# rpp0/gr-lora

Hardware: NVIDIA H100
Metric: LoRa symbols/s (dechirp+FFT+argmax) (higher is better)
Workload: dtype f32

## Files before the change

### gr_lora_b200/csrc/host_emul.cu

```cuda
#include "cuda_owned.h"
#include "k1_fft.cuh"
#include "k1_llr.cuh"
#include "k1_warp.cuh"
#include "k1_group.cuh"
#include "k1_sf10.cuh"
#include "k1_rows.cuh"
#include "int_chain.cuh"
#include "rx_stream.cuh"
#include "rx_sync.cuh"
#include "tx_channel.cuh"
#include "tx_encode.cuh"

#include <algorithm>
#include <cstring>
#include <vector>

template <int D>
static int k1_emulate_d(int sf, const lb::K1Args &a, uint32_t *bins, float *mags) {
    switch (sf) {
    case 7: lb::k1_emulate<7, D>(a, bins, mags); break;
    case 8: lb::k1_emulate<8, D>(a, bins, mags); break;
    case 9: lb::k1_emulate<9, D>(a, bins, mags); break;
    case 10: lb::k1_emulate<10, D>(a, bins, mags); break;
    case 11: lb::k1_emulate<11, D>(a, bins, mags); break;
    case 12: lb::k1_emulate<12, D>(a, bins, mags); break;
    default: return -1;
    }
    return 0;
}

template <int D>
static int k1_llr_emulate_d(int sf, const lb::K1Args &a, bool reduced, float *llrs, uint32_t *bins) {
    switch (sf) {
    case 7: lb::k1_llr_emulate<7, D>(a, reduced, llrs, bins); break;
    case 8: lb::k1_llr_emulate<8, D>(a, reduced, llrs, bins); break;
    case 9: lb::k1_llr_emulate<9, D>(a, reduced, llrs, bins); break;
    case 10: lb::k1_llr_emulate<10, D>(a, reduced, llrs, bins); break;
    case 11: lb::k1_llr_emulate<11, D>(a, reduced, llrs, bins); break;
    case 12: lb::k1_llr_emulate<12, D>(a, reduced, llrs, bins); break;
    default: return -1;
    }
    return 0;
}

extern "C" {

int lb_k1_emulate_osr(int sf, int osr, const float2 *x, size_t n_symbols, const float2 *chirp, const float2 *tw, uint32_t *bins,
                      float *mags) {
    const lb::K1Args a{x, chirp, tw, n_symbols};
    return osr == 8 ? k1_emulate_d<8>(sf, a, bins, mags) : osr == 2 ? k1_emulate_d<2>(sf, a, bins, mags) : -1;
}

int lb_k1_emulate(int sf, const float2 *x, size_t n_symbols, const float2 *chirp, const float2 *tw,
                  uint32_t *bins, float *mags) {
    return lb_k1_emulate_osr(sf, 8, x, n_symbols, chirp, tw, bins, mags);
}

int lb_k1_llr_emulate_osr(int sf, int osr, const float2 *x, size_t n_symbols, const float2 *chirp, const float2 *tw, int reduced,
                          float *llrs, uint32_t *bins) {
    const lb::K1Args a{x, chirp, tw, n_symbols};
    return osr == 8 ? k1_llr_emulate_d<8>(sf, a, reduced != 0, llrs, bins) : osr == 2 ? k1_llr_emulate_d<2>(sf, a, reduced != 0, llrs, bins) : -1;
}

int lb_k1_llr_emulate(int sf, const float2 *x, size_t n_symbols, const float2 *chirp, const float2 *tw, int reduced, float *llrs,
                      uint32_t *bins) {
    return lb_k1_llr_emulate_osr(sf, 8, x, n_symbols, chirp, tw, reduced, llrs, bins);
}

int lb_k1_emulate_warp_sf7(const float2 *x, size_t n_symbols, const float2 *chirp, const float2 *tw, uint32_t *bins, float *mags) {
    lb::K1Args a{x, chirp, tw, n_symbols};
    lb::w7_emulate(a, bins, mags);
    return 0;
}

int lb_k1_emulate_group(int sf, const float2 *x, size_t n_symbols, const float2 *chirp, const float2 *tw, uint32_t *bins, float *mags) {
    lb::K1Args a{x, chirp, tw, n_symbols};
    switch (sf) {
    case 8: lb::g_emulate<8>(a, bins, mags); break;
    case 9: lb::g_emulate<9>(a, bins, mags); break;
    case 10: lb::s10_emulate(a, bins, mags); break;
    default: return -1;
    }
    return 0;
}

int lb_k1_emulate_rows(int sf, const float2 *x, size_t n_symbols, const float2 *chirp, const float2 *tw, uint32_t *bins, float *mags) {
    lb::K1Args a{x, chirp, tw, n_symbols};
    if (sf == 11) lb::r_emulate<11>(a, bins, mags);
    else if (sf == 12) lb::r_emulate<12>(a, bins, mags);
    else return -1;
    return 0;
}


void lb_emul_philox4x32_10(const uint32_t *ctr, const uint32_t *key, uint32_t *out) {
    uint32_t c[4] = {ctr[0], ctr[1], ctr[2], ctr[3]};
    lb::philox4x32_10(c, key[0], key[1]);
    for (int i = 0; i < 4; i++) out[i] = c[i];
}

void lb_emul_atan2f(const float *y, const float *x, float *out, size_t n) {
    for (size_t i = 0; i < n; i++) out[i] = lb::lb_atan2f(y[i], x[i]);
}

uint32_t lb_emul_decode(const uint8_t *cw, uint32_t n_cw, int is_header, uint32_t cr, uint8_t *out, uint32_t cap) {
    uint32_t n = lb::decode_len_bytes(lb::decode_len_words(n_cw, is_header), cr);
    if (n > cap) n = cap;
    for (uint32_t i = 0; i < n; i++) out[i] = lb::decode_byte(cw, n_cw, is_header, cr, i);
    return n;
}
void lb_emul_deinterleave(const uint32_t *words, uint32_t n_words, uint32_t ppm, uint8_t *out) { lb::deinterleave_block(words, n_words, ppm, out); }
uint32_t lb_emul_reduce_bin(uint32_t bin, uint32_t n_hdr) { return lb::reduce_bin(bin, n_hdr); }
uint32_t lb_emul_gray(uint32_t bin) { return lb::gray_encode(bin); }
uint8_t lb_emul_hamming84_decode(uint8_t cw) { return lb::hamming84_decode(cw); }
uint8_t lb_emul_hamming84_encode(uint8_t v) { return lb::hamming84_encode(v); }
uint8_t lb_emul_deshuffle(uint8_t v) { return lb::deshuffle_byte(v); }
int32_t lb_emul_payload_symbols(uint32_t len, uint32_t cr, uint32_t sf, int rr) { return lb::payload_symbols(len, cr, sf, rr); }

uint32_t lb_emul_tx_encode(const uint8_t *payload, uint32_t len, uint32_t sf, uint32_t cr, int implicit, int crc, int reduced_rate,
                           uint32_t *shifts, uint32_t cap) {
    const lb::TxCode c{sf, cr, implicit ? 0u : 1u, crc ? 1u : 0u, reduced_rate ? 1u : 0u};
    if (!lb::tx_length_ok(c, len)) return 0;
    const uint32_t n = lb::tx_data_symbols(c, len);
    if (n > cap) return 0;
    for (uint32_t i = 0; i < n; i++) shifts[i] = lb::tx_symbol_shift(c, payload, len, i);
    return n;
}
uint32_t lb_emul_soft_header(uint32_t sf, uint32_t cr, int implicit, int crc, int reduced_rate, const float *llr, uint32_t *bins,
                             uint32_t *nib) {
    const lb::TxCode c{sf, cr, implicit ? 0u : 1u, crc ? 1u : 0u, reduced_rate ? 1u : 0u};
    return lb::rs_soft_header(c, llr, bins, nib).cr;
}
void lb_emul_soft_block(uint32_t sf, uint32_t cr, int implicit, int crc, int reduced_rate, uint32_t b, const float *llr, uint32_t *bins,
                        uint32_t *nib) {
    const lb::TxCode c{sf, cr, implicit ? 0u : 1u, crc ? 1u : 0u, reduced_rate ? 1u : 0u};
    lb::rs_soft_block(c, b, llr, bins, nib);
}
uint32_t lb_emul_header_checksum(uint32_t length, uint32_t cr, uint32_t crc) { return lb::header_checksum(length, cr, crc); }

uint32_t lb_emul_rx_replay(const int32_t *states, const float *metrics, const int32_t *bins, size_t n_steps, uint32_t sf,
                           int implicit, uint32_t cr, int crc, int reduced_rate, int32_t *next, lb::RxFrameRec *frames, uint32_t cap) {
    lb::RxParams p;
    memset(&p, 0, sizeof p);
    p.sf = sf; p.n_bins_hdr = 1u << (sf - 2); p.implicit = implicit; p.reduced_rate = reduced_rate;
    lb::RxStreamState st;
    lb::rx_state_init(&st, (uint8_t)(((cr & 7u) << 5) | (crc ? 1u << 4 : 0u)));
    uint32_t n_frames = 0;
    for (size_t i = 0; i < n_steps; i++) {
        const int s = states[i];
        next[i] = -1;
        if (s == LORA_B200_DETECT) next[i] = lb::rx_detect_commit(&st, 1.0f, 1.0f, 1u, metrics[i]);
        else if (s == LORA_B200_FIND_SFD) next[i] = lb::rx_sfd_commit(&st, metrics[i]);
        else if (s == LORA_B200_DECODE_HEADER || s == LORA_B200_DECODE_PAYLOAD) {
            const lb::RxSymbolResult r = lb::rx_symbol_commit(&st, p, s == LORA_B200_DECODE_HEADER, bins[i] >= 0, bins[i]);
            next[i] = r == lb::RX_HEADER_DONE ? LORA_B200_DECODE_PAYLOAD : r == lb::RX_FRAME_DONE ? LORA_B200_DETECT : s;
            if (r == lb::RX_FRAME_DONE) {
                if (n_frames < cap) {
                    lb::RxFrameRec *fr = frames + n_frames;
                    memcpy(fr->cw, st.demodulated, st.n_demod);
                    lb::rx_frame_record(fr, &st, 0, implicit);
                }
                n_frames++;
                lb::rx_frame_reset(&st);
            }
        }
    }
    return n_frames;
}
uint32_t lb_emul_rx_frame_rec_size(void) { return (uint32_t)sizeof(lb::RxFrameRec); }

}

namespace {

struct RsHostOps {
    const float2 *x;
    long long n_items;
    const float2 *down, *up, *tw;
    uint32_t sps, sf, osr;
    bool in_range(long long pos) const { return pos >= 0 && pos + (long long)sps <= n_items; }
    unsigned long long argmax(long long pos, bool use_up) {
        uint32_t b;
        float m;
        lb_k1_emulate_osr((int)sf, (int)osr, x + pos, 1, use_up ? up : down, tw, &b, &m);
        return lb::pack_key(m * m, b);
    }
    float2 binval(long long pos, float F, bool use_up, int bin) {
        const float2 *ch = use_up ? up : down;
        double re = 0.0, im = 0.0;
        for (uint32_t n = 0; n < sps; n++) {
            const double a = -2.0 * M_PI * ((double)F * (double)(pos + n) / sps + (double)bin * n / sps);
            const float2 v = lb::cmul(x[pos + n], ch[n]);
            re += v.x * cos(a) - v.y * sin(a);
            im += v.x * sin(a) + v.y * cos(a);
        }
        return make_float2((float)re, (float)im);
    }
    float energy(long long pos) {
        double e = 0.0;
        for (uint32_t n = 0; n < sps; n++) e += (double)x[pos + n].x * x[pos + n].x + (double)x[pos + n].y * x[pos + n].y;
        return (float)e;
    }
};

std::vector<float2> rs_host_windows(const RsHostOps &o, const lb::RsFrame &r, uint32_t first, uint32_t cnt) {
    std::vector<float2> w((size_t)cnt * o.sps);
    for (uint32_t k = 0; k < cnt; k++) {
        const long long s0 = lb::rs_sym(r.start, lb::rs_data_j((long long)first + k), o.sps, r.sfo_ppm);
        for (uint32_t i = 0; i < o.sps; i++) {
            const long long n = s0 + i;
            const double a = -2.0 * M_PI * (double)r.cfo_bins * (double)n / o.sps;
            const float2 v = o.x[n];
            w[(size_t)k * o.sps + i] = make_float2((float)(v.x * cos(a) - v.y * sin(a)), (float)(v.x * sin(a) + v.y * cos(a)));
        }
    }
    return w;
}

void rs_host_bins(const RsHostOps &o, const lb::RsFrame &r, uint32_t first, uint32_t cnt, std::vector<uint32_t> &bins) {
    const std::vector<float2> w = rs_host_windows(o, r, first, cnt);
    bins.resize(cnt);
    std::vector<float> mags(cnt);
    lb_k1_emulate_osr((int)o.sf, (int)o.osr, w.data(), cnt, o.down, o.tw, bins.data(), mags.data());
}

void rs_host_llrs(const RsHostOps &o, const lb::RsFrame &r, uint32_t first, uint32_t cnt, bool reduced, std::vector<float> &llr) {
    const std::vector<float2> w = rs_host_windows(o, r, first, cnt);
    llr.resize((size_t)cnt * (reduced ? o.sf - 2 : o.sf));
    lb_k1_llr_emulate_osr((int)o.sf, (int)o.osr, w.data(), cnt, o.down, o.tw, reduced, llr.data(), nullptr);
}

}

// ... 131 lines not shown
```

### gr_lora_b200/csrc/k1_sf10.cuh

```cuda
#pragma once
#include "k1_ring.cuh"

namespace lb {

constexpr int S10_T = 256, S10_N = 1024, S10_SPS = 8192;
constexpr int S10_SLOT_F2 = 8192;

struct S10Consts {
    float2 tl[4];
    float2 th[8];
    float2 wq[4];
};

LB_HD void s10_consts(int t, const float2 *tw, S10Consts &c) {
    const int a = t >> 3;
    for (int j = 0; j < 4; j++) c.tl[j] = k1_ld_table(tw + ((a * j * 8) & (S10_SPS - 1)));
    for (int j = 0; j < 8; j++) c.th[j] = k1_ld_table(tw + ((a * 4 * j * 8) & (S10_SPS - 1)));
    for (int i = 0; i < 4; i++) {
        const int q = t + S10_T * i;
        c.wq[i] = k1_ld_table(tw + ((q < S10_N / 2 ? q : q - S10_N) & (S10_SPS - 1)));
    }
}

LB_HD void s10_pass0_fft(const S10Consts &c, float2 *v);
LB_HD void s10_pass0(int t, const float2 *slot, const float2 *chirp, const S10Consts &c, float2 *v) {
#pragma unroll
    for (int r = 0; r < 32; r++) v[r] = cmul(slot[r * S10_T + t], chirp[r * S10_T + t]);
    s10_pass0_fft(c, v);
}
LB_HD void s10_pass0_fft(const S10Consts &c, float2 *v) {
    dft_dif<32>(v);
#pragma unroll
    for (int kc = 1; kc < 32; kc++) {
        const int br = bitrev<32>(kc);
        float2 w;
        if ((kc & 3) == 0) w = c.th[kc >> 2];
        else if ((kc >> 2) == 0) w = c.tl[kc & 3];
        else w = cmul(c.th[kc >> 2], c.tl[kc & 3]);
        v[br] = cmul(v[br], w);
    }
}

LB_HD void s10_store1(int t, float2 *slot, const float2 *v) {
#pragma unroll
    for (int kc = 0; kc < 32; kc++) slot[kc * S10_T + (t ^ ((kc & 1) << 3))] = v[bitrev<32>(kc)];
}

LB_HD void s10_pass1(int t, const float2 *slot, float2 *g) {
    const int kc = t >> 3, r = t & 7;
    const int sw = (kc & 1) << 3;
#pragma unroll
    for (int a = 0; a < 32; a++) g[a] = slot[kc * S10_T + ((a * 8 + r) ^ sw)];
    dft_dif<32>(g);
}

LB_HD int s10_pos2(int q, int r) { return q * 8 + ((((r >> 1) ^ ((q >> 1) & 3)) << 1) | (r & 1)); }

LB_HD void s10_store2(int t, float2 *slot, const float2 *g) {
    const int kc = t >> 3, r = t & 7;
#pragma unroll
    for (int ka = 0; ka < 32; ka++) slot[s10_pos2(kc + 32 * ka, r)] = g[bitrev<32>(ka)];
}

LB_HD unsigned long long s10_combine(int t, const float2 *slot, const S10Consts &c) {
    unsigned long long best = 0ull;
#pragma unroll
    for (int i = 0; i < 4; i++) {
        const int q = t + S10_T * i;
        float2 gv[8];
#pragma unroll
        for (int u = 0; u < 4; u++) {
            const float4 v = *reinterpret_cast<const float4 *>(slot + q * 8 + ((u ^ ((q >> 1) & 3)) << 1));
            gv[2 * u] = make_float2(v.x, v.y);
            gv[2 * u + 1] = make_float2(v.z, v.w);
        }
        float2 acc = horner<8>(gv, c.wq[i]);
        if (q == S10_N / 2) acc = plus_quirk<8>(acc, gv, c.wq[i]);
        const unsigned long long key = pack_key(cnorm2(acc), (uint32_t)q);
        best = key > best ? key : best;
    }
    return best;
}

#ifdef __CUDACC__
template <int NSLOT>
struct S10Smem {
    float2 chirp[S10_SLOT_F2];
    float2 slots[NSLOT][S10_SLOT_F2];
    uint64_t bars[NSLOT];
    unsigned long long keys[S10_T / 32];
};

template <int NSLOT>
__global__ void __launch_bounds__(S10_T, 1)
k1_sf10_kernel(K1Args a, uint32_t *__restrict__ bins, float *__restrict__ mags) {
    extern __shared__ __align__(128) unsigned char s10_raw[];
    S10Smem<NSLOT> &sm = *reinterpret_cast<S10Smem<NSLOT> *>(s10_raw);
    const int t = threadIdx.x, lane = t & 31, warp = t >> 5;
    const size_t g0 = blockIdx.x, g_total = gridDim.x;
    const SymbolRing<float2, S10_SLOT_F2, NSLOT> ring{sm.slots, sm.bars, a.x, g0, g_total, a.n_symbols};
    if (t == 0) ring.init();
    for (int i = t; i < S10_SLOT_F2; i += S10_T) sm.chirp[i] = k1_ld_table(a.chirp + i);
    __syncthreads();
    if (t == 0) ring.fill();
    S10Consts c;
    s10_consts(t, a.tw, c);
    uint32_t it = 0;
    for (size_t sym = g0; sym < a.n_symbols; sym += g_total, it++) {
        float2 *slot = ring.wait(it);
        float2 v[32];
        s10_pass0(t, slot, sm.chirp, c, v);
        __syncthreads();
        s10_store1(t, slot, v);
        __syncthreads();
        s10_pass1(t, slot, v);
        __syncthreads();
        s10_store2(t, slot, v);
        __syncthreads();
        unsigned long long best = s10_combine(t, slot, c);
        best = warp_max_key(best);
        if (lane == 0) sm.keys[warp] = best;
        __syncthreads();
        if (t == 0) {
            ring.refill(it, sym);
            unsigned long long bb = sm.keys[0];
#pragma unroll
            for (int k = 1; k < S10_T / 32; k++) bb = sm.keys[k] > bb ? sm.keys[k] : bb;
            k1_store(bins, mags, sym, bb);
        }
    }
}
#endif

inline void s10_emulate(const K1Args &a, uint32_t *bins, float *mags) {
    float2 *slot = new float2[S10_SLOT_F2];
    S10Consts *c = new S10Consts[S10_T];
    auto v = new float2[S10_T][32];
    for (int t = 0; t < S10_T; t++) s10_consts(t, a.tw, c[t]);
    for (size_t sym = 0; sym < a.n_symbols; sym++) {
        const float2 *x = a.x + sym * S10_SPS;
        for (int i = 0; i < S10_SLOT_F2; i++) slot[i] = x[i];
        for (int t = 0; t < S10_T; t++) s10_pass0(t, slot, a.chirp, c[t], v[t]);
        for (int i = 0; i < S10_SLOT_F2; i++) slot[i] = make_float2(NAN, NAN);
        for (int t = 0; t < S10_T; t++) s10_store1(t, slot, v[t]);
        for (int t = 0; t < S10_T; t++) s10_pass1(t, slot, v[t]);
        for (int i = 0; i < S10_SLOT_F2; i++) slot[i] = make_float2(NAN, NAN);
        for (int t = 0; t < S10_T; t++) s10_store2(t, slot, v[t]);
        unsigned long long best = 0ull;
        for (int t = 0; t < S10_T; t++) {
            const unsigned long long k = s10_combine(t, slot, c[t]);
            best = k > best ? k : best;
        }
        k1_store(bins, mags, sym, best);
    }
    delete[] slot; delete[] c; delete[] v;
}

}
```

### gr_lora_b200/csrc/lora_b200.cu

```cuda
#include "../../include/lora_b200.h"
#include "cuda_owned.h"
#include "k1_fft.cuh"
#include "k1_group.cuh"
#include "k1_sf10.cuh"
#include "k1_launch.h"
#include "rx_stream.cuh"
#include "rx_sync.cuh"
#include "rx_warp.cuh"
#include "tx_channel.cuh"
#include "tx_encode.cuh"

#include <algorithm>
#include <cmath>
#include <cstdarg>
#include <cstdio>
#include <cstring>
#include <cstdlib>
#include <memory>
#include <string>
#include <vector>

using namespace lb;

namespace {
// ... 36 lines not shown
    CudaEvent done;
    cudaStream_t last = nullptr;
};

constexpr uint32_t MAX_STAGE_GROUPS = 8;

}

struct lora_b200_decoder : A1Params {
    lora_b200_config cfg;
    uint32_t n_bins_hdr, decim;
    double bits_per_second, bits_per_symbol;
    bool k1_ok;
    bool k1_osr2;
    int device, n_sms;
    Tables toff;
    DeviceBuffer<uint8_t> d_tables;
    std::vector<uint8_t> h_tables;
    float down_ifreq_avg = 0.f, down_ifreq_sd = 0.f;
    K1Scratch k1s[3];
    DeviceBuffer<float> d_k2_scratch;
    int k2_grid = 0;
    CudaStream copy_streams[2];
    DeviceBuffer<float2> d_chunk[2];
    DeviceBuffer<short2> d_chunk16[2];
    PinnedBuffer<float2> h_chunk[2];
    DeviceBuffer<uint32_t> d_chunk_bins[2];
    DeviceBuffer<float> d_chunk_mags[2];
    CudaStream rx_stream, rx_stream2;
    CudaEvent rx2_done, rx_begin_ev;
    DeviceBuffer<RxStreamState> d_states;
    uint8_t phdr1_init = 0;
    DeviceBuffer<float> d_scratch;
    DeviceBuffer<unsigned long long> d_consumed;
    DeviceBuffer<RxFrameRec> d_frames;
    DeviceBuffer<RxFrameOut> d_frames_out;
    DeviceBuffer<uint32_t> d_n_frames;
    uint32_t frame_cap = 0;
    DeviceBuffer<lora_b200_step> d_trace;
    DeviceBuffer<uint32_t> d_trace_n;
    DeviceBuffer<float2> d_stage;
    DeviceBuffer<short2> d_stage16;
    PinnedBuffer<float2> h_stage;
    CudaEvent stage_events[MAX_STAGE_GROUPS];
    std::vector<unsigned long long> h_consumed;
    PinnedBuffer<RxFrameOut> h_frames;
    std::vector<RxFrameOut> h_sorted;
    std::vector<std::string> stdout_last;
    uint64_t launches = 0;
    bool cfo_estimate = false;
    DeviceBuffer<uint8_t> d_tx;
    CudaEvent tx_done;
    DeviceBuffer<float2> d_rs_stage, d_rs_win;
    DeviceBuffer<uint32_t> d_rs_bins[2], d_rs_hbins, d_rs_pbins, d_rs_ncand, d_rs_nframes, d_rs_tab;
    DeviceBuffer<float> d_rs_mags[2], d_rs_llr;
    DeviceBuffer<RsCand> d_rs_cands;
    DeviceBuffer<long long> d_rs_dropped;
    DeviceBuffer<unsigned long long> d_rs_hold;
    DeviceBuffer<RsFrame> d_rs_frames;
    DeviceBuffer<RxFrameRec> d_rs_recs;
    DeviceBuffer<RxFrameOut> d_rs_out;
    std::vector<lora_b200_rx_info> rs_info;
    uint32_t rs_hdr_drops = 0;
};

namespace {

void ifreq_host(const float2 *in, float *out, uint32_t window) {
    for (uint32_t i = 1u; i < window; i++) {
        const float p1 = atan2f(in[i - 1].y, in[i - 1].x);
        float p2 = atan2f(in[i].y, in[i].x);
        while ((p2 - p1) > M_PI) p2 = (float)(p2 - 2.0f * M_PI);
        while ((p2 - p1) < -M_PI) p2 = (float)(p2 + 2.0f * M_PI);
        out[i - 1] = p2 - p1;
    }
    out[window - 1] = out[window - 2];
}

Tables build_tables(const A1Params &p, uint32_t bandwidth, std::vector<uint8_t> &h) {
    const uint32_t sps = p.sps;
    Tables t;
    size_t o = 0;
    t.down = o; o += sizeof(float2) * sps;
    t.up = o; o += sizeof(float2) * sps;
    t.down_ifreq = o; o += sizeof(float) * sps;
    t.up_ifreq = o; o += sizeof(float) * sps;
    t.up_ifreq_v = o; o += sizeof(float) * sps * 3;
    t.tw = o; o += sizeof(float2) * sps;
    t.total = (o + 255) & ~(size_t)255;
    h.assign(t.total, 0);
    float2 *down = (float2 *)(h.data() + t.down);
    float2 *up = (float2 *)(h.data() + t.up);
    float *dif = (float *)(h.data() + t.down_ifreq);
    float *uif = (float *)(h.data() + t.up_ifreq);
    float *uifv = (float *)(h.data() + t.up_ifreq_v);
    float2 *tw = (float2 *)(h.data() + t.tw);

    const double T = -0.5 * bandwidth * p.symbols_per_second;
    const double f0 = bandwidth / 2.0;
    const double pre_dir = 2.0 * M_PI;
    for (uint32_t i = 0; i < sps; i++) {
        const double tt = p.dt * i;
        const float ph_d = (float)(pre_dir * tt * (f0 + T * tt));
        const float ph_u = (float)(pre_dir * tt * (f0 + T * tt) * -1.0f);
        const float cd = cosf(ph_d), sd = sinf(ph_d), cu = cosf(ph_u), su = sinf(ph_u);
        down[i] = make_float2(cd - sd, sd + cd);
        up[i] = make_float2(cu - su, su + cu);
    }
    ifreq_host(down, dif, sps);
    ifreq_host(up, uif, sps);
    std::vector<float2> tmp(3 * (size_t)sps);
    for (int k = 0; k < 3; k++) memcpy(tmp.data() + (size_t)k * sps, up, sizeof(float2) * sps);
    ifreq_host(tmp.data(), uifv, 3 * sps);
    for (uint32_t j = 0; j < sps; j++) {
        const double a = -2.0 * M_PI * (double)j / (double)sps;
        tw[j] = make_float2((float)cos(a), (float)sin(a));
    }
    return t;
}

void table_stats(const float *dif, uint32_t sps, float *avg_out, float *sd_out) {
    const uint32_t to_idx = sps - 1u;
    float acc = 0.0f;
    for (uint32_t i = 0; i < to_idx; i++) acc += dif[i];
    const float avg = acc / (float)to_idx;
    float var = 0.0f;
    for (uint32_t i = 0; i < to_idx; i++) { const float t = dif[i] - avg; var += t * t; }
    var /= (float)to_idx;
    *avg_out = avg;
    *sd_out = sqrtf(var);
}
void table_stats(lora_b200_decoder *d) { table_stats((const float *)(d->h_tables.data() + d->toff.down_ifreq), d->sps, &d->down_ifreq_avg, &d->down_ifreq_sd); }

template <typename T>
const T *tab(const lora_b200_decoder *d, size_t off) { return (const T *)(d->d_tables + off); }

int launched(lora_b200_decoder *d) { d->launches++; CU(cudaGetLastError()); return LORA_B200_OK; }

template <int SF, int D = 8>
int k1_launch_generic(const K1Launch &k) {
    using C = K1Cfg<SF, D>;
    static DeviceOnce once;
    const size_t smem = sizeof(float2) * C::SMEM_ELEMS;
    K1_CU(once(k.device, [&] { return cudaFuncSetAttribute(k1_fft_kernel<SF, D>, cudaFuncAttributeMaxDynamicSharedMemorySize, (int)smem); }));
    const size_t n_work = ((k.a.n_symbols + C::G - 1) / C::G) * C::S;
    const int grid = (int)std::min<size_t>(n_work, (size_t)k.n_sms * 2);
    k1_fft_kernel<SF, D><<<grid, K1_THREADS, smem, k.st>>>(k.a, k.bins, k.mags, k.packed);
    K1_CU(cudaGetLastError());
    return 0;
}

int k1_launch_sf10(const K1Launch &k) {
    static DeviceOnce once;
    const size_t smem = sizeof(S10Smem<2>);
    K1_CU(once(k.device, [&] { return cudaFuncSetAttribute(k1_sf10_kernel<2>, cudaFuncAttributeMaxDynamicSharedMemorySize, (int)smem); }));
    const int grid = (int)std::min<size_t>(k.a.n_symbols, (size_t)k.n_sms);
    k1_sf10_kernel<2><<<grid, S10_T, smem, k.st>>>(k.a, k.bins, k.mags);
    K1_CU(cudaGetLastError());
    return 0;
}

__global__ void k1_finalize_kernel(const unsigned long long *__restrict__ packed, size_t n, uint32_t *__restrict__ bins,
                                   float *__restrict__ mags) {
    const size_t i = blockIdx.x * (size_t)blockDim.x + threadIdx.x;
    if (i < n) k1_store(bins, mags, i, packed[i]);
}

bool k1_generic() {
    static int v = -1;
    if (v < 0) { const char *e = getenv("LORA_B200_K1"); v = e && !strcmp(e, "generic") ? 1 : 0; }
    return v == 1;
}

K1Launcher k1_launcher(int sf, bool generic) {
    switch (generic ? -sf : sf) {
    case 7: return k1_launch_warp7;
    case 8: return k1_launch_group<8, 6, 2>;
    case 9: return k1_launch_group9;
    case 10: return k1_launch_sf10;
    case 11: return k1_launch_rows<11>;
    case 12: return k1_launch_rows<12>;
    case -7: return k1_launch_generic<7>;
    case -8: return k1_launch_generic<8>;
    case -9: return k1_launch_generic<9>;
    case -10: return k1_launch_generic<10>;
    case -11: return k1_launch_generic<11>;
    case -12: return k1_launch_generic<12>;
    }
    return nullptr;
}

K1Launcher k1_launcher_osr2(int sf) {
    static_assert(K1Cfg<11, 2>::S == 1 && K1Cfg<12, 2>::S == 2, "k1_fft_kernel<SF, 2> splits SF12 only");
    switch (sf) {
    case 7: return k1_launch_generic<7, 2>;
    case 8: return k1_launch_generic<8, 2>;
    case 9: return k1_launch_generic<9, 2>;
    case 10: return k1_launch_generic<10, 2>;
    case 11: return k1_launch_generic<11, 2>;
    case 12: return k1_launch_generic<12, 2>;
    }
    return nullptr;
}

int dispatch_k1_impl(lora_b200_decoder *d, K1Scratch &ks, const float2 *iq, size_t n, uint32_t *bins, float *mags, cudaStream_t st) {
    if (!d->k1_ok && !d->k1_osr2) return fail(LORA_B200_EUNSUPPORTED, "FFT demodulator needs samp_rate/bandwidth == 8 or 2 and SF7..SF12");
    if (n == 0) return LORA_B200_OK;
    static const char *rows = getenv("LORA_B200_K1_ROWS");
    const int sf = (int)d->cfg.sf;
    const bool generic = k1_generic() || (sf >= 11 && rows && rows[0] == '0');
    const K1Launcher launch = d->k1_osr2 ? k1_launcher_osr2(sf) : k1_launcher(sf, generic);
    if (!launch) return fail(LORA_B200_EUNSUPPORTED, "unsupported SF %u", d->cfg.sf);
    const bool split = sf == 12 || (sf == 11 && generic && !d->k1_osr2);
    if (split) {
        CU(ks.packed.reserve(n));
        CU(cudaMemsetAsync(ks.packed, 0, sizeof(unsigned long long) * n, st));
    }
    char err[256] = {0};
    const K1Launch k{K1Args{iq, tab<float2>(d, d->toff.down), tab<float2>(d, d->toff.tw), n},
                     (const float2 *)(d->h_tables.data() + d->toff.tw), bins, mags, split ? ks.packed.get() : nullptr,
                     d->device, d->n_sms, st, err, sizeof err};
    if (launch(k)) return fail(LORA_B200_ECUDA, "K1: %s", err);
    d->launches++;
    if (split) {
        k1_finalize_kernel<<<(unsigned)((n + 255) / 256), 256, 0, st>>>(ks.packed, n, bins, mags);
        if (int rc = launched(d)) return rc;
    }
    return LORA_B200_OK;
}

int dispatch_k1(lora_b200_decoder *d, K1Scratch &ks, const float2 *iq, size_t n, uint32_t *bins, float *mags, cudaStream_t st) {
    CU(ks.done.ensure());
    if (ks.last != st) CU(cudaStreamWaitEvent(st, ks.done, 0));
    const int rc = dispatch_k1_impl(d, ks, iq, n, bins, mags, st);
    if (rc) return rc;
    CU(cudaEventRecord(ks.done, st));
    ks.last = st;
    return LORA_B200_OK;
}

template <int SF, int D>
int llr_launch(lora_b200_decoder *d, const float2 *iq, size_t n, bool reduced, float *llrs, uint32_t *bins, cudaStream_t st) {
    using C = K1Cfg<SF, D>;
    static DeviceOnce once;
    const size_t smem = sizeof(float2) * C::SMEM_ELEMS;
    CU(once(d->device, [&] { return cudaFuncSetAttribute(k1_llr_kernel<SF, D>, cudaFuncAttributeMaxDynamicSharedMemorySize, (int)smem); }));
    const size_t n_batches = (n + C::G - 1) / C::G;
    const int grid = (int)std::min<size_t>(n_batches, (size_t)d->n_sms * 2);
    k1_llr_kernel<SF, D><<<grid, K1_THREADS, smem, st>>>(K1Args{iq, tab<float2>(d, d->toff.down), tab<float2>(d, d->toff.tw), n},
                                                         reduced ? 1 : 0, llrs, bins);
    return launched(d);
}

template <int D>
int dispatch_llr_d(lora_b200_decoder *d, const float2 *iq, size_t n, bool reduced, float *llrs, uint32_t *bins, cudaStream_t st) {
    switch (d->cfg.sf) {
    case 7: return llr_launch<7, D>(d, iq, n, reduced, llrs, bins, st);
    case 8: return llr_launch<8, D>(d, iq, n, reduced, llrs, bins, st);
    case 9: return llr_launch<9, D>(d, iq, n, reduced, llrs, bins, st);
    case 10: return llr_launch<10, D>(d, iq, n, reduced, llrs, bins, st);
    case 11: return llr_launch<11, D>(d, iq, n, reduced, llrs, bins, st);
    case 12: return llr_launch<12, D>(d, iq, n, reduced, llrs, bins, st);
    }
    return fail(LORA_B200_EUNSUPPORTED, "unsupported SF %u", d->cfg.sf);
}

int dispatch_llr(lora_b200_decoder *d, const float2 *iq, size_t n, bool reduced, float *llrs, uint32_t *bins, cudaStream_t st) {
    if (!d->k1_ok && !d->k1_osr2) return fail(LORA_B200_EUNSUPPORTED, "the LLR demodulator needs samp_rate/bandwidth == 8 or 2 and SF7..SF12");
    if (n == 0) return LORA_B200_OK;
    return d->k1_osr2 ? dispatch_llr_d<2>(d, iq, n, reduced, llrs, bins, st) : dispatch_llr_d<8>(d, iq, n, reduced, llrs, bins, st);
}

template <int SF, bool FFT>
int launch_rx_t(lora_b200_decoder *d, const RxParams &p, int grid, cudaStream_t st) {
    size_t smem = 0;
    if (FFT) {
        smem = sizeof(float2) * K1Cfg<SF>::SMEM_ELEMS;
        static DeviceOnce once;
        CU(once(d->device, [&] { return cudaFuncSetAttribute(rx_stream_kernel<SF, FFT>, cudaFuncAttributeMaxDynamicSharedMemorySize, (int)smem); }));
    }
    rx_stream_kernel<SF, FFT><<<grid, RX_THREADS, smem, st>>>(p);
    return launched(d);
}

bool rx_warp_path(const lora_b200_decoder *d) { return d->cfg.sf == 7 && d->sps == (uint32_t)RW_SPS && d->n_bins == (uint32_t)RW_N; }

template <bool FFT>
int launch_rx_warp(lora_b200_decoder *d, const RxParams &p, int n_streams, cudaStream_t st) {
    static DeviceOnce once;
    const size_t smem = sizeof(RWSmem);
    CU(once(d->device, [&] { return cudaFuncSetAttribute(rx_warp_kernel<FFT>, cudaFuncAttributeMaxDynamicSharedMemorySize, (int)smem); }));
    rx_warp_kernel<FFT><<<(n_streams + RW_WARPS - 1) / RW_WARPS, RW_WARPS * 32, smem, st>>>(p);
    return launched(d);
}

int launch_rx(lora_b200_decoder *d, const RxParams &p, int grid, cudaStream_t st) {
    const bool fft = d->cfg.demod == LORA_B200_DEMOD_FFT;
    if (rx_warp_path(d)) return fft ? launch_rx_warp<true>(d, p, grid, st) : launch_rx_warp<false>(d, p, grid, st);
    if (!fft) return launch_rx_t<7, false>(d, p, grid, st);
    switch (d->cfg.sf) {
    case 8: return launch_rx_t<8, true>(d, p, grid, st);
    case 9: return launch_rx_t<9, true>(d, p, grid, st);
    case 10: return launch_rx_t<10, true>(d, p, grid, st);
    case 11: return launch_rx_t<11, true>(d, p, grid, st);
    case 12: return launch_rx_t<12, true>(d, p, grid, st);
    }
    return fail(LORA_B200_EUNSUPPORTED, "unsupported SF %u", d->cfg.sf);
}

void append_hex(std::string &s, const uint8_t *v, size_t n, bool endline, bool ascii) {
// ... 998 lines not shown
```

Baseline: 363.3 million.

## Restructure SF10 kernel to 512 threads with warp-local FFT passes

Rewrites the SF10 dechirp+FFT+argmax kernel from 256 threads doing a 32x32 split to 512 threads doing 16x16x4 stages. The chirp moves from shared memory into registers, and the later passes become warp-local, using __syncwarp and shuffles instead of block-wide barriers. The ring grows to three slots, and the key reduction and refill for each symbol are deferred into the next iteration so they overlap with compute. This is meant to cut block-level synchronisation and shared-memory traffic, at the cost of more registers per thread and more complex indexing and quirk handling.

Result: no change. 362.9 million (median of 6 runs) (-0.1%).

```diff
diff --git a/gr_lora_b200/csrc/host_emul.cu b/gr_lora_b200/csrc/host_emul.cu
--- a/gr_lora_b200/csrc/host_emul.cu
+++ b/gr_lora_b200/csrc/host_emul.cu
@@ -78,7 +78,7 @@
     switch (sf) {
     case 8: lb::g_emulate<8>(a, bins, mags); break;
     case 9: lb::g_emulate<9>(a, bins, mags); break;
-    case 10: lb::s10_emulate(a, bins, mags); break;
+    case 10: lb::k10_emulate(a, bins, mags); break;
     default: return -1;
     }
     return 0;
diff --git a/gr_lora_b200/csrc/k1_sf10.cuh b/gr_lora_b200/csrc/k1_sf10.cuh
--- a/gr_lora_b200/csrc/k1_sf10.cuh
+++ b/gr_lora_b200/csrc/k1_sf10.cuh
@@ -3,157 +3,207 @@
 
 namespace lb {
 
-constexpr int S10_T = 256, S10_N = 1024, S10_SPS = 8192;
-constexpr int S10_SLOT_F2 = 8192;
-
-struct S10Consts {
-    float2 tl[4];
-    float2 th[8];
+constexpr int K10_T = 512, K10_N = 1024, K10_SPS = 8192, K10_NSLOT = 3;
+
+struct K10Consts {
+    float2 tl[3];
+    float2 th[3];
+    float2 wc[3];
     float2 wq[4];
+    float2 w4[2];
 };
 
-LB_HD void s10_consts(int t, const float2 *tw, S10Consts &c) {
-    const int a = t >> 3;
-    for (int j = 0; j < 4; j++) c.tl[j] = k1_ld_table(tw + ((a * j * 8) & (S10_SPS - 1)));
-    for (int j = 0; j < 8; j++) c.th[j] = k1_ld_table(tw + ((a * 4 * j * 8) & (S10_SPS - 1)));
+LB_HD int k10_signed(int k) { return k < K10_N / 2 ? k : k - K10_N; }
+
+LB_HD void k10_consts(int t, const float2 *tw, K10Consts &c) {
+    const int b = t >> 5, lane = t & 31, K = (t >> 5) + 16 * (lane >> 1), h = lane & 1;
+    for (int j = 1; j < 4; j++) {
+        c.tl[j - 1] = k1_ld_table(tw + ((32 * b * j) & (K10_SPS - 1)));
+        c.th[j - 1] = k1_ld_table(tw + ((128 * b * j) & (K10_SPS - 1)));
+        c.wc[j - 1] = k1_ld_table(tw + ((8 * j * K) & (K10_SPS - 1)));
+    }
+    for (int kq = 0; kq < 4; kq++) {
+        const int ks = k10_signed(K + 256 * kq);
+        c.wq[kq] = k1_ld_table(tw + (ks & (K10_SPS - 1)));
+        if ((kq >> 1) == h) c.w4[kq & 1] = k1_ld_table(tw + ((4 * ks) & (K10_SPS - 1)));
+    }
+}
+
+LB_HD void k10_chirp(int t, const float2 *chirp, float2 *ch) {
+    for (int j = 0; j < 16; j++) ch[j] = k1_ld_table(chirp + 512 * j + t);
+}
+
+LB_HD void k10_pass0(int t, float2 *slot, const float2 *ch, const K10Consts &c) {
+    float2 v[16];
+#pragma unroll
+    for (int j = 0; j < 16; j++) v[j] = cmul(slot[512 * j + t], ch[j]);
+    dft_dif<16>(v);
+#pragma unroll
+    for (int kc = 0; kc < 16; kc++) {
+        const int lo = kc & 3, hi = kc >> 2;
+        float2 o = v[bitrev<16>(kc)];
+        if (lo && hi) o = cmul(o, cmul(c.th[hi - 1], c.tl[lo - 1]));
+        else if (lo) o = cmul(o, c.tl[lo - 1]);
+        else if (hi) o = cmul(o, c.th[hi - 1]);
+        slot[512 * kc + t] = o;
+    }
+}
+
+LB_HD int k10_swz(int kb) { return (kb & 1) | ((kb & 2) << 1); }
+LB_HD int k10_word(int kc, int kb, int l) { return 512 * kc + 32 * kb + ((((l >> 1) ^ k10_swz(kb)) << 1) | (l & 1)); }
+
+LB_HD void k10_pass1_load(int t, const float2 *slot, float2 *v) {
+    const int kc = t >> 5, l = t & 31;
+#pragma unroll
+    for (int b = 0; b < 16; b++) v[b] = slot[512 * kc + 32 * b + l];
+    dft_dif<16>(v);
+}
+LB_HD void k10_pass1_store(int t, float2 *slot, const float2 *v) {
+    const int kc = t >> 5, l = t & 31;
+#pragma unroll
+    for (int kb = 0; kb < 16; kb++) slot[k10_word(kc, kb, l)] = v[bitrev<16>(kb)];
+}
+
+LB_HD void k10_pass2(int t, const float2 *slot, const K10Consts &c, float2 *T, float2 &Tq) {
+    const int kc = t >> 5, lane = t & 31, kb = lane >> 1, h = lane & 1;
+    float2 g[4][4];
+#pragma unroll
+    for (int cc = 0; cc < 4; cc++)
+#pragma unroll
+        for (int e = 0; e < 2; e++) {
+            const float4 u = *reinterpret_cast<const float4 *>(slot + k10_word(kc, kb, 8 * cc + 4 * h + 2 * e));
+            g[2 * e][cc] = make_float2(u.x, u.y);
+            g[2 * e + 1][cc] = make_float2(u.z, u.w);
+        }
+#pragma unroll
     for (int i = 0; i < 4; i++) {
-        const int q = t + S10_T * i;
-        c.wq[i] = k1_ld_table(tw + ((q < S10_N / 2 ? q : q - S10_N) & (S10_SPS - 1)));
-    }
-}
-
-LB_HD void s10_pass0_fft(const S10Consts &c, float2 *v);
-LB_HD void s10_pass0(int t, const float2 *slot, const float2 *chirp, const S10Consts &c, float2 *v) {
-#pragma unroll
-    for (int r = 0; r < 32; r++) v[r] = cmul(slot[r * S10_T + t], chirp[r * S10_T + t]);
-    s10_pass0_fft(c, v);
-}
-LB_HD void s10_pass0_fft(const S10Consts &c, float2 *v) {
-    dft_dif<32>(v);
-#pragma unroll
-    for (int kc = 1; kc < 32; kc++) {
-        const int br = bitrev<32>(kc);
-        float2 w;
-        if ((kc & 3) == 0) w = c.th[kc >> 2];
-        else if ((kc >> 2) == 0) w = c.tl[kc & 3];
-        else w = cmul(c.th[kc >> 2], c.tl[kc & 3]);
-        v[br] = cmul(v[br], w);
-    }
-}
-
-LB_HD void s10_store1(int t, float2 *slot, const float2 *v) {
-#pragma unroll
-    for (int kc = 0; kc < 32; kc++) slot[kc * S10_T + (t ^ ((kc & 1) << 3))] = v[bitrev<32>(kc)];
-}
-
-LB_HD void s10_pass1(int t, const float2 *slot, float2 *g) {
-    const int kc = t >> 3, r = t & 7;
-    const int sw = (kc & 1) << 3;
-#pragma unroll
-    for (int a = 0; a < 32; a++) g[a] = slot[kc * S10_T + ((a * 8 + r) ^ sw)];
-    dft_dif<32>(g);
-}
-
-LB_HD int s10_pos2(int q, int r) { return q * 8 + ((((r >> 1) ^ ((q >> 1) & 3)) << 1) | (r & 1)); }
-
-LB_HD void s10_store2(int t, float2 *slot, const float2 *g) {
-    const int kc = t >> 3, r = t & 7;
-#pragma unroll
-    for (int ka = 0; ka < 32; ka++) slot[s10_pos2(kc + 32 * ka, r)] = g[bitrev<32>(ka)];
-}
-
-LB_HD unsigned long long s10_combine(int t, const float2 *slot, const S10Consts &c) {
+#pragma unroll
+        for (int cc = 1; cc < 4; cc++) g[i][cc] = cmul(g[i][cc], c.wc[cc - 1]);
+        dft_dif<4>(g[i]);
+    }
+    Tq = make_float2(0.0f, 0.0f);
+#pragma unroll
+    for (int kq = 0; kq < 4; kq++) {
+        float2 gv[4];
+#pragma unroll
+        for (int i = 0; i < 4; i++) gv[i] = g[i][bitrev<4>(kq)];
+        T[kq] = horner<4>(gv, c.wq[kq]);
+        if (kq == 2 && kc == 0 && kb == 0) Tq = horner<4>(gv, cconj(c.wq[2]));
+    }
+}
+
+LB_HD float2 k10_keep(int h, const float2 *T, int i) { return h ? T[2 + i] : T[i]; }
+LB_HD float2 k10_give(int h, const float2 *T, int i) { return h ? T[i] : T[2 + i]; }
+
+LB_HD unsigned long long k10_key(int t, const K10Consts &c, const float2 *T, const float2 *got, float2 Tq, float2 tq_got) {
+    const int lane = t & 31, K = (t >> 5) + 16 * (lane >> 1), h = lane & 1;
     unsigned long long best = 0ull;
 #pragma unroll
-    for (int i = 0; i < 4; i++) {
-        const int q = t + S10_T * i;
-        float2 gv[8];
-#pragma unroll
-        for (int u = 0; u < 4; u++) {
-            const float4 v = *reinterpret_cast<const float4 *>(slot + q * 8 + ((u ^ ((q >> 1) & 3)) << 1));
-            gv[2 * u] = make_float2(v.x, v.y);
-            gv[2 * u + 1] = make_float2(v.z, v.w);
-        }
-        float2 acc = horner<8>(gv, c.wq[i]);
-        if (q == S10_N / 2) acc = plus_quirk<8>(acc, gv, c.wq[i]);
-        const unsigned long long key = pack_key(cnorm2(acc), (uint32_t)q);
+    for (int i = 0; i < 2; i++) {
+        const float2 own = k10_keep(h, T, i), hi = h ? own : got[i], lo = h ? got[i] : own;
+        float2 f = cfma(hi, c.w4[i], lo);
+        if (i == 0 && h && K == 0) f = cadd(f, cfma(Tq, cconj(c.w4[0]), tq_got));
+        const unsigned long long key = pack_key(cnorm2(f), (uint32_t)(K + 256 * (2 * h + i)));
         best = key > best ? key : best;
     }
     return best;
 }
 
 #ifdef __CUDACC__
-template <int NSLOT>
-struct S10Smem {
-    float2 chirp[S10_SLOT_F2];
-    float2 slots[NSLOT][S10_SLOT_F2];
-    uint64_t bars[NSLOT];
-    unsigned long long keys[S10_T / 32];
+struct K10Smem {
+    float2 slots[K10_NSLOT][K10_SPS];
+    uint64_t bars[K10_NSLOT];
+    unsigned long long keys[2][K10_T / 32];
 };
 
-template <int NSLOT>
-__global__ void __launch_bounds__(S10_T, 1)
+__global__ void __launch_bounds__(K10_T, 1)
 k1_sf10_kernel(K1Args a, uint32_t *__restrict__ bins, float *__restrict__ mags) {
-    extern __shared__ __align__(128) unsigned char s10_raw[];
-    S10Smem<NSLOT> &sm = *reinterpret_cast<S10Smem<NSLOT> *>(s10_raw);
+    extern __shared__ __align__(128) unsigned char k10_raw[];
+    K10Smem &sm = *reinterpret_cast<K10Smem *>(k10_raw);
     const int t = threadIdx.x, lane = t & 31, warp = t >> 5;
     const size_t g0 = blockIdx.x, g_total = gridDim.x;
-    const SymbolRing<float2, S10_SLOT_F2, NSLOT> ring{sm.slots, sm.bars, a.x, g0, g_total, a.n_symbols};
+    const SymbolRing<float2, K10_SPS, K10_NSLOT> ring{sm.slots, sm.bars, a.x, g0, g_total, a.n_symbols};
     if (t == 0) ring.init();
-    for (int i = t; i < S10_SLOT_F2; i += S10_T) sm.chirp[i] = k1_ld_table(a.chirp + i);
     __syncthreads();
     if (t == 0) ring.fill();
-    S10Consts c;
-    s10_consts(t, a.tw, c);
+    float2 ch[16];
+    k10_chirp(t, a.chirp, ch);
+    K10Consts c;
+    k10_consts(t, a.tw, c);
+    auto finish = [&](uint32_t it, size_t sym) {
+        unsigned long long k = lane < K10_T / 32 ? sm.keys[it & 1][lane] : 0ull;
+        k = warp_max_key(k);
+        if (lane == 0) k1_store(bins, mags, sym, k);
+    };
     uint32_t it = 0;
-    for (size_t sym = g0; sym < a.n_symbols; sym += g_total, it++) {
+    size_t sym = g0;
+    for (; sym < a.n_symbols; sym += g_total, it++) {
         float2 *slot = ring.wait(it);
-        float2 v[32];
-        s10_pass0(t, slot, sm.chirp, c, v);
+        k10_pass0(t, slot, ch, c);
         __syncthreads();
-        s10_store1(t, slot, v);
-        __syncthreads();
-        s10_pass1(t, slot, v);
-        __syncthreads();
-        s10_store2(t, slot, v);
-        __syncthreads();
-        unsigned long long best = s10_combine(t, slot, c);
+        if (it > 0 && warp == 0) {
+            if (lane == 0) ring.refill(it - 1, sym - g_total);
+            finish(it - 1, sym - g_total);
+        }
+        {
+            float2 v[16];
+            k10_pass1_load(t, slot, v);
+            __syncwarp();
+            k10_pass1_store(t, slot, v);
+        }
+        __syncwarp();
+        float2 T[4], Tq, got[2];
+        k10_pass2(t, slot, c, T, Tq);
+        const int h = lane & 1;
+#pragma unroll
+        for (int i = 0; i < 2; i++) {
+            const float2 s = k10_give(h, T, i);
+            got[i].x = __shfl_xor_sync(0xffffffffu, s.x, 1);
+            got[i].y = __shfl_xor_sync(0xffffffffu, s.y, 1);
+        }
+        float2 tq_got = make_float2(0.0f, 0.0f);
+        if (warp == 0) {
+            tq_got.x = __shfl_xor_sync(0xffffffffu, Tq.x, 1);
+            tq_got.y = __shfl_xor_sync(0xffffffffu, Tq.y, 1);
+        }
+        unsigned long long best = k10_key(t, c, T, got, Tq, tq_got);
         best = warp_max_key(best);
-        if (lane == 0) sm.keys[warp] = best;
-        __syncthreads();
-        if (t == 0) {
-            ring.refill(it, sym);
-            unsigned long long bb = sm.keys[0];
-#pragma unroll
-            for (int k = 1; k < S10_T / 32; k++) bb = sm.keys[k] > bb ? sm.keys[k] : bb;
-            k1_store(bins, mags, sym, bb);
-        }
-    }
+        if (lane == 0) sm.keys[it & 1][warp] = best;
+    }
+    __syncthreads();
+    if (it > 0 && warp == 0) finish(it - 1, sym - g_total);
 }
 #endif
 
-inline void s10_emulate(const K1Args &a, uint32_t *bins, float *mags) {
-    float2 *slot = new float2[S10_SLOT_F2];
-    S10Consts *c = new S10Consts[S10_T];
-    auto v = new float2[S10_T][32];
-    for (int t = 0; t < S10_T; t++) s10_consts(t, a.tw, c[t]);
+inline void k10_emulate(const K1Args &a, uint32_t *bins, float *mags) {
+    float2 *slot = new float2[K10_SPS];
+    K10Consts *c = new K10Consts[K10_T];
+    auto ch = new float2[K10_T][16];
+    auto v = new float2[K10_T][16];
+    auto T = new float2[K10_T][4];
+    float2 *Tq = new float2[K10_T];
+    for (int t = 0; t < K10_T; t++) {
+        k10_consts(t, a.tw, c[t]);
+        k10_chirp(t, a.chirp, ch[t]);
+    }
     for (size_t sym = 0; sym < a.n_symbols; sym++) {
-        const float2 *x = a.x + sym * S10_SPS;
-        for (int i = 0; i < S10_SLOT_F2; i++) slot[i] = x[i];
-        for (int t = 0; t < S10_T; t++) s10_pass0(t, slot, a.chirp, c[t], v[t]);
-        for (int i = 0; i < S10_SLOT_F2; i++) slot[i] = make_float2(NAN, NAN);
-        for (int t = 0; t < S10_T; t++) s10_store1(t, slot, v[t]);
-        for (int t = 0; t < S10_T; t++) s10_pass1(t, slot, v[t]);
-        for (int i = 0; i < S10_SLOT_F2; i++) slot[i] = make_float2(NAN, NAN);
-        for (int t = 0; t < S10_T; t++) s10_store2(t, slot, v[t]);
+        const float2 *x = a.x + sym * K10_SPS;
+        for (int i = 0; i < K10_SPS; i++) slot[i] = x[i];
+        for (int t = 0; t < K10_T; t++) k10_pass0(t, slot, ch[t], c[t]);
+        for (int t = 0; t < K10_T; t++) k10_pass1_load(t, slot, v[t]);
+        for (int i = 0; i < K10_SPS; i++) slot[i] = make_float2(NAN, NAN);
+        for (int t = 0; t < K10_T; t++) k10_pass1_store(t, slot, v[t]);
+        for (int t = 0; t < K10_T; t++) k10_pass2(t, slot, c[t], T[t], Tq[t]);
         unsigned long long best = 0ull;
-        for (int t = 0; t < S10_T; t++) {
-            const unsigned long long k = s10_combine(t, slot, c[t]);
+        for (int t = 0; t < K10_T; t++) {
+            const int h = t & 1;
+            const float2 got[2] = {k10_give(1 - h, T[t ^ 1], 0), k10_give(1 - h, T[t ^ 1], 1)};
+            const unsigned long long k = k10_key(t, c[t], T[t], got, Tq[t], Tq[t ^ 1]);
             best = k > best ? k : best;
         }
         k1_store(bins, mags, sym, best);
     }
-    delete[] slot; delete[] c; delete[] v;
-}
-
-}
+    delete[] slot; delete[] c; delete[] ch; delete[] v; delete[] T; delete[] Tq;
+}
+
+}
diff --git a/gr_lora_b200/csrc/lora_b200.cu b/gr_lora_b200/csrc/lora_b200.cu
--- a/gr_lora_b200/csrc/lora_b200.cu
+++ b/gr_lora_b200/csrc/lora_b200.cu
@@ -212,10 +212,10 @@
 
 int k1_launch_sf10(const K1Launch &k) {
     static DeviceOnce once;
-    const size_t smem = sizeof(S10Smem<2>);
-    K1_CU(once(k.device, [&] { return cudaFuncSetAttribute(k1_sf10_kernel<2>, cudaFuncAttributeMaxDynamicSharedMemorySize, (int)smem); }));
+    const size_t smem = sizeof(K10Smem);
+    K1_CU(once(k.device, [&] { return cudaFuncSetAttribute(k1_sf10_kernel, cudaFuncAttributeMaxDynamicSharedMemorySize, (int)smem); }));
     const int grid = (int)std::min<size_t>(k.a.n_symbols, (size_t)k.n_sms);
-    k1_sf10_kernel<2><<<grid, S10_T, smem, k.st>>>(k.a, k.bins, k.mags);
+    k1_sf10_kernel<<<grid, K10_T, smem, k.st>>>(k.a, k.bins, k.mags);
     K1_CU(cudaGetLastError());
     return 0;
 }
```
